# bamler-lab/constriction

Hardware: AMD Instinct MI355X
Metric: Msymbols/s encode+decode, 64k x 4k-symbol streams, bit-exact vs CPU (higher is better)
Workload: dtype u64; 1 GPU; C2: 65536 streams/GPU x 4096 int32 symbols (stream-major), shared 12-bit QuantizedGaussian(-50,50,3.2,9.6), AnsCoder (W,S,P)=(32,64,12), encode into slabs + decode; u64 coder state, u32 words, i32 symbols; streams_per_gpu=65536, parallelism=streams sharded over 1 GPU(s), no data-path collective

## Files before the change

constriction_amd/csrc/cst_family_policy.hpp:

```cpp
#pragma once
#include "cst_math.hpp"
#include "cst_family_math.hpp"

namespace cst {

__device__ __forceinline__ float ndtri_lower_f32(float tail) {
    constexpr float a1 = -3.969683028665376e+01f, a2 = 2.209460984245205e+02f, a3 = -2.759285104469687e+02f, a4 = 1.383577518672690e+02f,
        a5 = -3.066479806614716e+01f, a6 = 2.506628277459239e+00f, b1 = -5.447609879822406e+01f, b2 = 1.615858368580409e+02f,
        b3 = -1.556989798598866e+02f, b4 = 6.680131188771972e+01f, b5 = -1.328068155288572e+01f, c1 = -7.784894002430293e-03f,
        c2 = -3.223964580411365e-01f, c3 = -2.400758277161838e+00f, c4 = -2.549732539343734e+00f, c5 = 4.374664141464968e+00f,
        c6 = 2.938163982698783e+00f, d1 = 7.784695709041462e-03f, d2 = 3.224671290700398e-01f, d3 = 2.445134137142996e+00f,
        d4 = 3.754408661907416e+00f;
    auto f = [](float a, float b, float c) { return __builtin_fmaf(a, b, c); };
    const float q = __builtin_amdgcn_sqrtf(-1.3862943611f * __builtin_amdgcn_logf(tail));
    const float zt = f(f(f(f(f(c1, q, c2), q, c3), q, c4), q, c5), q, c6) * __builtin_amdgcn_rcpf(f(f(f(f(d1, q, d2), q, d3), q, d4), q, 1.0f));
    const float u = tail - 0.5f, r = u * u;
    const float zc = f(f(f(f(f(a1, r, a2), r, a3), r, a4), r, a5), r, a6) * u * __builtin_amdgcn_rcpf(f(f(f(f(f(b1, r, b2), r, b3), r, b4), r, b5), r, 1.0f));
    return tail < 0.02425f ? zt : zc;
}

__device__ __forceinline__ float ndtri_lower_coarse_f32(float tail) {
    const float t = __builtin_amdgcn_sqrtf(-1.3862943611f * __builtin_amdgcn_logf(tail));
    const float num = __builtin_fmaf(__builtin_fmaf(0.010328f, t, 0.802853f), t, 2.515517f);
    const float den = __builtin_fmaf(__builtin_fmaf(__builtin_fmaf(0.001308f, t, 0.189269f), t, 1.432788f), t, 1.0f);
    return __builtin_fmaf(num, __builtin_amdgcn_rcpf(den), -t);
}

__device__ __forceinline__ bool family_params_valid(double a, double b) {
    return b > 0.0 && b <= 1.7976931348623157e308 && fabs(a) <= 1.7976931348623157e308;
}

struct GaussianFamily {
    static constexpr bool kGaussian = true, kErfTab = true;
    __device__ static __forceinline__ bool valid(double mu, double sd) { return family_params_valid(mu, sd); }
    __device__ static __forceinline__ bool lcp(int32_t sym, int32_t lo, int32_t hi, int P, double mu, double sd, uint32_t& left, uint32_t& prob,
                                               const double2* tab) {
        return leaky_gaussian_lcp_quick(sym, lo, hi, P, 32, mu, sd, left, prob, tab);
    }
    template <bool INNER = false>
    __device__ static __forceinline__ uint32_t left(int32_t i, int32_t lo, int32_t n, int P, double mu, double sd, const double2* tab) {
        return leaky_gaussian_left_quick<INNER>(i, lo, n, P, 32, mu, sd, tab);
    }
    __device__ static __forceinline__ void left3(uint32_t g, int32_t lo, uint32_t n, int P, double mu, double sd, const double2* tab, uint32_t (&v)[3]) {
        leaky_gaussian_left3_quick(g, lo, n, P, mu, sd, tab, v);
    }
    __device__ static __forceinline__ float guess_z(float tail) { return ndtri_lower_f32(tail); }
    __device__ static __forceinline__ float guess_z_coarse(float tail) { return ndtri_lower_coarse_f32(tail); }
};

static __device__ __attribute__((noinline)) double laplace_left_f64(double x, double mu, double b, double free_weight) {
    return free_weight * laplace_cdf_exact(x, mu, b);
}
static __device__ __attribute__((noinline)) double cauchy_left_f64(double x, double x0, double gamma, double free_weight) {
    return free_weight * cauchy_cdf_exact(x, x0, gamma);
}

template <class CDF>
struct ExactFamily {
    static constexpr bool kGaussian = false, kErfTab = false;
    __device__ static __forceinline__ bool valid(double a, double b) { return family_params_valid(a, b); }
    __device__ static __forceinline__ uint32_t total(int P) { return P >= 32 ? 0u : (1u << P); }
    __device__ static __forceinline__ uint32_t value(uint32_t i, int32_t lo, uint32_t n, int P, double a, double b) {
        const double free_weight = (double)((total(P) - 1u) - (n - 1u));
        const double x = (double)(int32_t)((uint32_t)lo + i) - 0.5;
        return f64_as_u32_hw(CDF::left_f64(x, a, b, free_weight));
    }
    template <bool INNER = false>
    __device__ static __forceinline__ uint32_t left(int32_t i, int32_t lo, int32_t n, int P, double a, double b, const double2*) {
        if constexpr (!INNER) {
            if (i <= 0) return 0u;
            if (i >= n) return total(P);
        }
        return value((uint32_t)i, lo, (uint32_t)n, P, a, b) + (uint32_t)i;
    }
    __device__ static __forceinline__ void left3(uint32_t g, int32_t lo, uint32_t n, int P, double a, double b, const double2*, uint32_t (&v)[3]) {
#pragma unroll 1
        for (uint32_t k = 0; k < 3; ++k) {
            const uint32_t i = g - 1u + k;
            const uint32_t ic = min(max(i, 1u), n - 1u);
            const uint32_t val = value(ic, lo, n, P, a, b) + ic;
            const uint32_t r = i == 0u ? 0u : i >= n ? total(P) : val;
            if (k == 0) v[0] = r; else if (k == 1) v[1] = r; else v[2] = r;
        }
    }
    __device__ static __forceinline__ bool lcp(int32_t sym, int32_t lo, int32_t hi, int P, double a, double b, uint32_t& left_out, uint32_t& prob,
                                               const double2*) {
        const bool inside = sym >= lo && sym <= hi;
        const uint32_t n = (uint32_t)hi - (uint32_t)lo + 1u;
        const uint32_t i = inside ? (uint32_t)sym - (uint32_t)lo : 0u;
        uint32_t e[2];
#pragma unroll 1
        for (uint32_t k = 0; k < 2; ++k) {
            const uint32_t j = i + k;
            const uint32_t jc = min(max(j, 1u), n - 1u);
            const uint32_t val = value(jc, lo, n, P, a, b) + jc;
            const uint32_t r = j == 0u ? 0u : j >= n ? total(P) : val;
            if (k == 0) e[0] = r; else e[1] = r;
        }
        left_out = e[0];
        prob = e[1] - e[0];
        return inside;
    }
    __device__ static __forceinline__ float guess_z(float tail) { return CDF::z(tail); }
    __device__ static __forceinline__ float guess_z_coarse(float tail) { return CDF::z(tail); }
};

struct LaplaceCdf {
    __device__ static __forceinline__ double left_f64(double x, double mu, double b, double fw) { return laplace_left_f64(x, mu, b, fw); }
    __device__ static __forceinline__ float z(float tail) { return 0.69314718f * __builtin_amdgcn_logf(2.0f * tail); }
};
struct CauchyCdf {
    __device__ static __forceinline__ double left_f64(double x, double x0, double g, double fw) { return cauchy_left_f64(x, x0, g, fw); }
    __device__ static __forceinline__ float z(float tail) {
        const float pt = 3.14159265f * tail;
        const float far = __builtin_fmaf(pt, -0.33333333f, __builtin_amdgcn_rcpf(pt));
        const float near = __builtin_amdgcn_cosf(0.5f * tail) * __builtin_amdgcn_rcpf(__builtin_amdgcn_sinf(0.5f * tail));
        return -(tail < 0.03125f ? far : near);
    }
};
using LaplaceFamily = ExactFamily<LaplaceCdf>;
using CauchyFamily = ExactFamily<CauchyCdf>;

}
```

constriction_amd/csrc/cst_math.hpp:

```cpp
#pragma once
#include <hip/hip_runtime.h>
#include <stdint.h>

namespace cst {

__device__ __forceinline__ uint32_t f64_hi(double x) { return (uint32_t)__double2hiint(x); }
__device__ __forceinline__ uint32_t f64_lo(double x) { return (uint32_t)__double2loint(x); }
__device__ __forceinline__ double f64_from(uint32_t lo, uint32_t hi) { return __hiloint2double((int)hi, (int)lo); }
__device__ __forceinline__ double f64_clear_lo(double x) { return __hiloint2double(__double2hiint(x), 0); }
__device__ __forceinline__ double f64_pow2(int n) { return __hiloint2double((0x3ff + n) << 20, 0); }

__device__ inline double scalbn_exact(double x, int n) {
    double y = x;
    if (n > 1023) {
        y *= 0x1p1023; n -= 1023;
        if (n > 1023) { y *= 0x1p1023; n -= 1023; if (n > 1023) n = 1023; }
    } else if (n < -1022) {
        y *= 0x1p-1022 * 0x1p53; n += 1022 - 53;
        if (n < -1022) { y *= 0x1p-1022 * 0x1p53; n += 1022 - 53; if (n < -1022) n = -1022; }
    }
    return y * f64_pow2(n);
}

__device__ inline double exp_exact(double x) {
// ... 247 lines not shown
}

template <bool TAB = false>
__device__ __forceinline__ uint32_t leaky_gaussian_left(int32_t i, int32_t lo, int32_t n, int P, int prob_bits, double mu,
                                                        double sigma, const double2* tab = nullptr) {
    const uint32_t pmask = prob_bits >= 32 ? 0xffffffffu : ((1u << prob_bits) - 1u);
    if (i <= 0) return 0u;
    if (i >= n) return (P >= 32 ? 0u : (1u << P)) & pmask;
    const uint32_t max_prob = pmask >> (prob_bits - P);
    const double free_weight = (double)(max_prob - (uint32_t)(n - 1));
    const double x = (double)(int32_t)((uint32_t)lo + (uint32_t)i) - 0.5;
    return (f64_as_u32_sat(free_weight * gaussian_cdf_exact<TAB>(x, mu, sigma, tab)) + (uint32_t)i) & pmask;
}

static __device__ __attribute__((noinline)) double leaky_left_f64_exact(double x, double mu, double sigma, double free_weight, const double2* tab) {
    constexpr double sqrt2 = 1.41421356237309504880168872420969808;
    return free_weight * ((1.0 + erf_exact_tab((x - mu) / (sigma * sqrt2), tab)) / 2.0);
}

__device__ __forceinline__ uint32_t leaky_left_value_quick(double x, double mu, double sigma, double inv_d, double free_weight,
                                                           const double2* tab, uint32_t* n_exact) {
    constexpr double sqrt2 = 1.41421356237309504880168872420969808;
    const double arg = (x - mu) * inv_d;
    const double half = 0.5 * free_weight;
    double y = __builtin_fma(erf_fast_poly(arg, tab), half, half);
    const double fr = __builtin_amdgcn_fract(y);
    const bool same = __builtin_fabs(arg) >= 6.0;
    const bool sure = __builtin_fabs(fr - 0.5) < 0.5 - kLeftGuard;
    const bool unsure = !(same || sure);
    if (__builtin_amdgcn_ballot_w64(unsure) != 0ull) {
        if (unsure) {
            y = leaky_left_f64_exact(x, mu, sigma, free_weight, tab);
            if (n_exact) ++*n_exact;
        }
    }
    return f64_as_u32_hw(y);
}

template <bool INNER = false>
__device__ __forceinline__ uint32_t leaky_gaussian_left_quick(int32_t i, int32_t lo, int32_t n, int P, int prob_bits, double mu,
                                                              double sigma, const double2* tab, uint32_t* n_exact = nullptr) {
    constexpr double sqrt2 = 1.41421356237309504880168872420969808;
    const uint32_t pmask = prob_bits >= 32 ? 0xffffffffu : ((1u << prob_bits) - 1u);
    if constexpr (!INNER) {
        if (i <= 0) return 0u;
        if (i >= n) return (P >= 32 ? 0u : (1u << P)) & pmask;
    }
    const uint32_t max_prob = pmask >> (prob_bits - P);
    const double free_weight = (double)(max_prob - (uint32_t)(n - 1));
    const double x = (double)(int32_t)((uint32_t)lo + (uint32_t)i) - 0.5;
    return (leaky_left_value_quick(x, mu, sigma, fast_rcp1(sigma * sqrt2), free_weight, tab, n_exact) + (uint32_t)i) & pmask;
}

__device__ __forceinline__ void leaky_gaussian_left3_quick(uint32_t g, int32_t lo, uint32_t n, int P, double mu, double sigma,
                                                           const double2* tab, uint32_t (&v)[3]) {
    constexpr double sqrt2 = 1.41421356237309504880168872420969808;
    const uint32_t total = P >= 32 ? 0u : (1u << P);
    const double free_weight = (double)((total - 1u) - (n - 1u));
    const double half = 0.5 * free_weight;
    const double inv_d = fast_rcp1(sigma * sqrt2);
    const double x1 = (double)(int32_t)((uint32_t)lo + g) - 0.5;
    const double x[3] = {x1 - 1.0, x1, x1 + 1.0};
    double y[3], arg[3];
    bool unsure[3];
    ErfPoly e[3];
#pragma unroll
    for (int k = 0; k < 3; ++k) {
        arg[k] = (x[k] - mu) * inv_d;
        e[k] = erf_poly_fetch(arg[k], tab);
    }
    __builtin_amdgcn_sched_barrier(0);
#pragma unroll
    for (int k = 0; k < 3; ++k) {
        y[k] = __builtin_fma(erf_poly_eval(e[k], arg[k]), half, half);
        unsure[k] = !(__builtin_fabs(arg[k]) >= 6.0 || __builtin_fabs(__builtin_amdgcn_fract(y[k]) - 0.5) < 0.5 - kLeftGuard);
    }
    unsure[0] = unsure[0] && g > 1u;
    unsure[2] = unsure[2] && g + 1u < n;
    if (__builtin_amdgcn_ballot_w64(unsure[0] || unsure[1] || unsure[2]) != 0ull) {
#pragma unroll
        for (int k = 0; k < 3; ++k)
            if (unsure[k]) y[k] = leaky_left_f64_exact(x[k], mu, sigma, free_weight, tab);
    }
    v[0] = g > 1u ? f64_as_u32_hw(y[0]) + (g - 1u) : 0u;
    v[1] = f64_as_u32_hw(y[1]) + g;
    v[2] = g + 1u < n ? f64_as_u32_hw(y[2]) + (g + 1u) : total;
}

__device__ __forceinline__ bool leaky_gaussian_lcp_quick(int32_t sym, int32_t lo, int32_t hi, int P, int prob_bits, double mu, double sigma,
                                                         uint32_t& left, uint32_t& prob, const double2* tab) {
    constexpr double sqrt2 = 1.41421356237309504880168872420969808;
    const bool inside = sym >= lo && sym <= hi;
    const int32_t sc = inside ? sym : lo;
    const uint32_t pmask = prob_bits >= 32 ? 0xffffffffu : ((1u << prob_bits) - 1u);
    const uint32_t max_prob = pmask >> (prob_bits - P);
    const double free_weight = (double)(max_prob - ((uint32_t)hi - (uint32_t)lo));
    const double half = 0.5 * free_weight;
    const uint32_t slack = ((uint32_t)sc - (uint32_t)lo) & pmask;
    const double inv_d = fast_rcp1(sigma * sqrt2);
    const double xl = (double)sc - 0.5, xr = (double)sc + 0.5;
    const double al = (xl - mu) * inv_d, ar = (xr - mu) * inv_d;
    const ErfPoly el = erf_poly_fetch(al, tab), er = erf_poly_fetch(ar, tab);
    __builtin_amdgcn_sched_barrier(0);
    double yl = __builtin_fma(erf_poly_eval(el, al), half, half), yr = __builtin_fma(erf_poly_eval(er, ar), half, half);
    const bool unsure_l = !(__builtin_fabs(al) >= 6.0 || __builtin_fabs(__builtin_amdgcn_fract(yl) - 0.5) < 0.5 - kLeftGuard) && sc != lo;
    const bool unsure_r = !(__builtin_fabs(ar) >= 6.0 || __builtin_fabs(__builtin_amdgcn_fract(yr) - 0.5) < 0.5 - kLeftGuard) && sc != hi;
    if (__builtin_amdgcn_ballot_w64(unsure_l || unsure_r) != 0ull) {
#pragma unroll 1
        for (int side = 0; side < 2; ++side) {
            const bool u = side ? unsure_r : unsure_l;
            if (__builtin_amdgcn_ballot_w64(u) == 0ull) continue;
            if (u) {
                const double y = leaky_left_f64_exact(side ? xr : xl, mu, sigma, free_weight, tab);
                if (side) yr = y; else yl = y;
            }
        }
    }
    const uint32_t l = sc == lo ? 0u : (f64_as_u32_hw(yl) + slack) & pmask;
    const uint32_t r = sc == hi ? ((P >= 32 ? 0u : (1u << P)) & pmask) : (f64_as_u32_hw(yr) + slack + 1u) & pmask;
    left = l;
    prob = (r - l) & pmask;
    return inside;
}

}
```

constriction_amd/csrc/cst_persymbol.hip:

```cpp
#include <cstdlib>
#include <mutex>

#include "cst_persymbol.hpp"

namespace cst {

__global__ void cp_entries_kernel(const uint32_t* __restrict__ left, const uint32_t* __restrict__ prob, size_t n, int P,
                                  EncEntry* __restrict__ out) {
    const size_t i = (size_t)blockIdx.x * blockDim.x + threadIdx.x;
    if (i >= n) return;
    uint32_t c = left[i], p = prob[i];
    if ((uint64_t)c + p > ((uint64_t)1 << P)) p = 0;
    out[i] = make_entry(c, p);
}

template <int W, int S, int KIND>
__global__ __launch_bounds__(kBlock) void encode_entries_kernel(const EntriesEncodeArgs a) {
    extern __shared__ __attribute__((aligned(16))) unsigned char smem[];
    const int lane = threadIdx.x & (kWave - 1);
    uint32_t* ring = reinterpret_cast<uint32_t*>(smem) + (threadIdx.x >> 6) * kRingWords;
    const size_t s = (size_t)blockIdx.x * blockDim.x + threadIdx.x;
    const bool active = s < a.n_streams;
    const size_t N = a.n_per_stream;
    const int P = a.precision;
// ... 264 lines not shown
}

__device__ __noinline__ void store_symbol_tile16(int32_t* sym, size_t n_streams, size_t N, size_t s0, size_t t0, int lane, const int32_t* tile, bool vec) {
#pragma unroll
    for (int k = 0; k < 4; ++k) {
        const size_t r = (size_t)(lane >> 2) + 16 * k;
        if (s0 + r >= n_streams) continue;
        const int32_t* src = tile + r * 20 + 4 * (lane & 3);
        int32_t* dst = sym + (s0 + r) * N + t0 + 4 * (lane & 3);
        if (vec) {
            const int4 v = *reinterpret_cast<const int4*>(src);
            v4i t; t.x = v.x; t.y = v.y; t.z = v.z; t.w = v.w;
            __builtin_nontemporal_store(t, reinterpret_cast<v4i*>(dst));
        } else {
            dst[0] = src[0]; dst[1] = src[1]; dst[2] = src[2]; dst[3] = src[3];
        }
    }
}

template <class PT> __device__ __forceinline__ size_t edge_row_length(size_t n) {
    if constexpr (kParamF32<PT>) asm volatile("" : "+s"(n));
    return n;
}

template <int W, int S, int KIND, bool SMALL = false, class FAM = GaussianFamily, class PT = double>
__global__ __launch_bounds__(LaneGeo<SMALL>::kThreads) void decode_gaussian_lane_kernel(const PerSymbolDecodeArgs a) {
    using G = LaneGeo<SMALL>;
    constexpr int kParTile = G::kParTile, kWordWindow = G::kWordWindow, kOutSyms = G::kOutSyms, kOutStride = G::kOutStride;
    constexpr size_t kLaneDecWaveBytes = G::kWaveBytes;
    extern __shared__ __attribute__((aligned(16))) unsigned char smem[];
    double2* erf_tab = reinterpret_cast<double2*>(smem);
    if constexpr (FAM::kErfTab) {
        erf_tab_fill(erf_tab, threadIdx.x, blockDim.x);
        __syncthreads();
    }
    const int lane = threadIdx.x & (kWave - 1);
    unsigned char* mine = smem + (FAM::kErfTab ? kErfTabBytes : 0) + (size_t)(threadIdx.x >> 6) * kLaneDecWaveBytes;
    int32_t* tile = reinterpret_cast<int32_t*>(mine);
    double* par_mu = reinterpret_cast<double*>(mine + (size_t)kWave * kOutStride * 4);
    double* par_sd = par_mu + kParTile * kParStride;
    uint32_t* win = reinterpret_cast<uint32_t*>(par_sd + kParTile * kParStride);
    const size_t s = (size_t)blockIdx.x * blockDim.x + threadIdx.x;
    const size_t s0 = s - lane;
    if (s0 >= a.n_streams) return;
    const bool active = s < a.n_streams;
    const size_t se = active ? s : a.n_streams - 1;
    const size_t N = a.n_per_stream;
    const int P = a.precision;
    const bool raw = (a.flags & CST_FLAG_RAW_STATE) != 0;
    const uint32_t n = (uint32_t)a.n_symbols;
    const bool symbol_major = a.layout == CST_LAYOUT_SYMBOL_MAJOR;
    const size_t stride_t = symbol_major ? a.n_streams : 1;
    const size_t e0 = symbol_major ? se : se * N;
    const double free_weight = (double)((P >= 32 ? 0xffffffffu : ((1u << P) - 1u)) - (n - 1u));
    const float total_f = (float)(1ull << P), free_f = (float)free_weight, inv_total_f = 1.0f / total_f, inv_free_f = 1.0f / free_f;
    const double guess_shift = 0.5 - (double)a.min_symbol;
    const bool vec = !symbol_major && (N % 4 == 0) && (reinterpret_cast<uintptr_t>(a.symbols) & 15) == 0;
    const bool two_step_guess = (double)n * 64.0 > free_weight;

    DirectDecoder<W, S, KIND> D;
    D.init(a, se, raw);
    int32_t status = D.status;
    int32_t* sym_p = a.symbols + e0;

    constexpr int kVec = !kParamF32<PT> ? 1 : SMALL ? 2 : KIND != kRange ? 4 : 1;
    constexpr int kReqTile = kParamsPerLine<PT>;
    constexpr int kReqParts = kReqTile / kParTile;
    constexpr bool kMulti = kReqParts > 1;
    PT mu_r[kReqTile], sd_r[kReqTile];
    const PT* const means = params_as<PT>(a.means);
    const PT* const stds = params_as<PT>(a.stds);
    int mode = 0;
    const size_t base_e = symbol_major ? s0 + (size_t)lane : (s0 + (size_t)(lane / kParTile)) * N + (size_t)(lane % kParTile);
    const size_t t_stride = symbol_major ? a.n_streams : 1, item_stride = symbol_major ? a.n_streams : (size_t)(kWave / kParTile) * N;
    const int base_l = symbol_major ? lane : (lane % kParTile) * kParStride + lane / kParTile;
    const int l_stride = symbol_major ? kParStride : kWave / kParTile;
    const bool vec_ok = kVec == 1 || (N % kVec == 0 && ((reinterpret_cast<uintptr_t>(means) | reinterpret_cast<uintptr_t>(stds)) & (4 * kVec - 1)) == 0);
    const bool pairs = kMulti && !symbol_major && s0 + kWave <= a.n_streams && vec_ok;
    constexpr int kLanesPerRow = kReqTile / kVec;
    typedef float vec_t __attribute__((ext_vector_type(kVec > 1 ? kVec : 2)));
    auto par_request = [&](size_t t0) {
        if (kMulti && pairs && t0 % kReqTile == 0 && t0 + kReqTile <= N) {
            if constexpr (kVec > 1) {
                const size_t ev = (s0 + (size_t)(lane / kLanesPerRow)) * N + (size_t)(kVec * (lane % kLanesPerRow)) + t0;
#pragma unroll
                for (int it = 0; it < kLanesPerRow; ++it) {
                    const vec_t mv = __builtin_nontemporal_load(reinterpret_cast<const vec_t*>(means + ev + (size_t)it * (kWave / kLanesPerRow) * N));
                    const vec_t sv = __builtin_nontemporal_load(reinterpret_cast<const vec_t*>(stds + ev + (size_t)it * (kWave / kLanesPerRow) * N));
#pragma unroll
                    for (int c = 0; c < kVec; ++c) { mu_r[kVec * it + c] = mv[c]; sd_r[kVec * it + c] = sv[c]; }
                }
                mode = 1;
                return;
            }
            const size_t e = (s0 + (size_t)(lane / kReqTile)) * N + (size_t)(lane % kReqTile) + t0;
            const PT* pm = means + e;
            const PT* ps = stds + e;
#pragma unroll
            for (int it = 0; it < kReqTile; ++it) {
                mu_r[it] = __builtin_nontemporal_load(pm + (size_t)it * (size_t)(kWave / kReqTile) * N);
                sd_r[it] = __builtin_nontemporal_load(ps + (size_t)it * (size_t)(kWave / kReqTile) * N);
            }
            mode = 1;
            return;
        }
        mode = 0;
        if (s0 + kWave <= a.n_streams && t0 + kParTile <= N) {
            const PT* pm = means + base_e + t0 * t_stride;
            const PT* ps = stds + base_e + t0 * t_stride;
#pragma unroll
            for (int it = 0; it < kParTile; ++it) {
// ... 45 lines not shown
            par_mu[base_l + it * l_stride] = (double)mu_r[it];
            par_sd[base_l + it * l_stride] = (double)sd_r[it];
        }
    };
    uint32_t w_r[kParTile];
    int64_t w_first = 0;
    auto win_request = [&](int64_t first) {
        w_first = first;
        const int64_t len = (int64_t)D.length();
        if (!__any(first < 0 || first + kParTile > len)) {
            const uint32_t* pw = D.in + first;
#pragma unroll
            for (int i = 0; i < kParTile; ++i) w_r[i] = pw[i];
            return;
        }
#pragma unroll
        for (int i = 0; i < kParTile; ++i) {
            const int64_t p = first + i;
            w_r[i] = *(p >= 0 && p < len ? D.in + p : D.idle);
        }
    };
    auto win_land = [&]() {
#pragma unroll
        for (int i = 0; i < kParTile; ++i) win[(((uint32_t)(w_first + i)) & (kWordWindow - 1)) * kWave + lane] = w_r[i];
    };
    const auto window_of = [&](int ahead_tiles) -> int64_t {
        return D.kDownward ? (int64_t)D.position() - (int64_t)kParTile * (ahead_tiles + 1) : (int64_t)D.position() + (int64_t)kParTile * ahead_tiles;
    };

    if (N > 0) {
        par_request(0);
        win_request(window_of(0));
    }
    for (size_t t0 = 0; t0 < N; t0 += kParTile) {
        wave_lds_fence();
        par_land();
        win_land();
        if (t0 + kParTile < N && mode == 0) par_request(t0 + kParTile);
        win_request(window_of(1));
        wave_lds_fence();
        const int n_here = (int)(N - t0 < (size_t)kParTile ? N - t0 : (size_t)kParTile);
#pragma unroll 1
        for (int tl = 0; tl < n_here; ++tl) {
            const size_t t = t0 + (size_t)tl;
            int32_t sym = 0;
            const double mu = par_mu[tl * kParStride + lane], sd = par_sd[tl * kParStride + lane];
            D.ahead = win[(((uint32_t)D.next_index()) & (kWordWindow - 1)) * kWave + lane];
            if (status == CST_STREAM_OK) {
                const bool model_ok = FAM::valid(mu, sd);
                const uint32_t q = model_ok ? D.quantile(P) : 0u;
                if (!model_ok) status = CST_STREAM_IMPOSSIBLE_SYMBOL;
                else if (D.status != CST_STREAM_OK) status = D.status;
                else {
                    const float below = (float)q + 0.5f, above = total_f - below;
                    const bool coarse = FAM::kGaussian && !__any(sd >= 200.0);
                    float z = coarse ? FAM::guess_z_coarse(fminf(below, above) * inv_total_f) : FAM::guess_z(fminf(below, above) * inv_total_f);
                    double x = mu + sd * (double)(below < above ? z : -z) + guess_shift;
                    if (two_step_guess) {
                        const float b1 = below - (float)fmin(fmax(x, 0.0), (double)(n - 1u)), a1 = free_f - b1;
                        z = FAM::guess_z(fmaxf(fminf(b1, a1), 0.25f) * inv_free_f);
                        x = mu + sd * (double)(b1 < a1 ? z : -z) + guess_shift;
                    }
                    const uint32_t g = (uint32_t)fmin(fmax(x + 0.5, 1.0), (double)(n - 1u));
                    uint32_t lo_i = 0, hi_i = n, lo_v = 0, hi_v = P >= 32 ? 0u : (1u << P);
                    uint32_t probe = g, step = 1;
                    bool up = false, down = false;
                    {
                        uint32_t v3[3];
                        FAM::left3(g, a.min_symbol, n, P, mu, sd, erf_tab, v3);
                        if (v3[1] <= q) {
                            up = true;
                            if (q < v3[2]) { lo_i = g; lo_v = v3[1]; hi_i = g + 1u; hi_v = v3[2]; }
                            else { lo_i = g + 1u; lo_v = v3[2]; probe = min(g + 2u, n - 1u); step = 2; }
                        } else {
                            down = true;
                            if (v3[0] <= q) { lo_i = g - 1u; lo_v = v3[0]; hi_i = g; hi_v = v3[1]; }
                            else { hi_i = g - 1u; hi_v = v3[0]; probe = max(g - 1u, 2u) - 1u; step = 2; }
                        }
                    }
                    while (hi_i - lo_i > 1) {
                        const uint32_t v = FAM::template left<true>((int32_t)probe, a.min_symbol, (int32_t)n, P, mu, sd, erf_tab);
                        if (v <= q) { lo_i = probe; lo_v = v; up = true; } else { hi_i = probe; hi_v = v; down = true; }
                        if (up && down) probe = lo_i + (hi_i - lo_i) / 2;
                        else if (up) probe = min(lo_i + step, hi_i - 1u);
                        else probe = max(hi_i - min(step, hi_i - 1u), lo_i + 1u);
                        step *= 2;
                    }
                    const uint32_t c = lo_v, p = hi_v - lo_v;
                    if (p == 0 || c > q || (uint64_t)c + p > ((uint64_t)1 << P)) status = CST_STREAM_IMPOSSIBLE_SYMBOL;
                    else {
                        sym = a.min_symbol + (int32_t)lo_i;
                        D.advance(q, c, p, P);
                    }
                }
            }
            if (symbol_major) {
                if (active) *sym_p = sym;
                sym_p += stride_t;
            } else {
                tile[lane * kOutStride + (t % kOutSyms)] = sym;
                if (t % kOutSyms == kOutSyms - 1) {
                    wave_lds_fence();
                    if constexpr (SMALL) store_symbol_tile16(a.symbols, a.n_streams, N, s0, t - (kOutSyms - 1), lane, tile, vec);
                    else store_symbol_tile(a.symbols, a.n_streams, N, s0, t - (kOutSyms - 1), lane, tile, vec);
                    wave_lds_fence();
                }
            }
        }
    }
    if (!symbol_major) {
        const size_t done = N - N % kOutSyms;
        if (active) for (size_t t = done; t < N; ++t) a.symbols[se * N + t] = tile[lane * kOutStride + (t % kOutSyms)];
    }
    if (!active) return;
    a.status[s] = status;
    D.finish(a, s, raw);
}

constexpr int kRowsAhead = 16;

template <class FAM = GaussianFamily, class PT = double>
__global__ __launch_bounds__(kRowEntries) void gaussian_rows_kernel(int P, int32_t lo, int32_t n, const PT* __restrict__ means,
                                                                   const PT* __restrict__ stds, int32_t layout, size_t n_streams,
                                                                   size_t N, size_t t0, size_t count, uint32_t* __restrict__ rows) {
    const double2* erf_tab = nullptr;
    if constexpr (FAM::kErfTab) {
        __shared__ double2 erf_lds[kErfTabEntries];
        erf_tab_fill(erf_lds, threadIdx.x, blockDim.x);
        __syncthreads();
        erf_tab = erf_lds;
    }
    const size_t row = blockIdx.x;
    const size_t s = row / count, t = t0 + row % count;
    const size_t e = layout == CST_LAYOUT_SYMBOL_MAJOR ? t * n_streams + s : s * N + t;
    const double mu = load_param(means + e), sd = load_param(stds + e);
    const int32_t i = (int32_t)threadIdx.x;
    const uint32_t total = 1u << P;
    uint32_t v;
    if (FAM::valid(mu, sd))
        v = i <= n ? FAM::template left<false>(i, lo, n, P, mu, sd, erf_tab) : total;
    else v = i == 0 ? 0xffffffffu : total;
    rows[row * kRowEntries + i] = v;
}

// ... 891 lines not shown
```

constriction_amd/csrc/cst_persymbol.hpp:

```cpp
#pragma once
#include <type_traits>

#include "cst_range_kernels.hpp"
#include "cst_math.hpp"
#include "cst_family_policy.hpp"

namespace cst {

enum CoderKind : int { kAns = 0, kRange = 1, kChain = 2 };

template <class PT> __device__ __forceinline__ const PT* params_as(const void* p) { return static_cast<const PT*>(p); }
template <class PT> __device__ __forceinline__ double load_param(const PT* p) { return (double)*p; }
template <class PT> inline constexpr bool kParamF32 = std::is_same_v<PT, float>;
template <class PT> inline constexpr int kParamsPerLine = 128 / (int)sizeof(PT);

inline const float* f32(const void* p) { return static_cast<const float*>(p); }

__device__ __forceinline__ EncEntry make_entry(uint32_t c, uint32_t p) {
    uint64_t m = 0;
    if (p == 1) m = ~0ull;
    else if (p > 1) {
        const uint64_t q = (~0ull) / p;
        const uint64_t r = (~0ull) - q * p;
        m = q + ((r + 1 == p) ? 1 : 0);
    }
    return EncEntry{c, p, (uint32_t)m, (uint32_t)(m >> 32)};
}

struct EntriesEncodeArgs {
    const EncEntry* entries;
    size_t n_streams, n_per_stream;
    int32_t layout, precision;
    uint32_t* words;
    size_t stride_words;
    uint32_t* n_words;
    uint64_t* state;
    cst_range_state* rstate;
    int32_t* status;
    uint32_t flags;
    const uint32_t* pop_words; const uint64_t* pop_offsets; size_t pop_stride; uint32_t* n_pop;
    cst_chain_heads* heads;
};

constexpr int kEntryGroup = 8;

constexpr int kFuTile = 16;
constexpr int kFuStreams = 32;
constexpr int kFuIters = kFuTile * kFuStreams / kWave;
constexpr int kFuRingSlots = 32;
constexpr int kFuAhead = 4;
constexpr int kFuRowStride = kFuStreams + 1;
constexpr int kFuBlock = 256;
constexpr size_t kFuTabBytes = kErfTabBytes;
constexpr size_t kFuWaveBytes = (size_t)kFuRingSlots * kWave * 4 + (size_t)kFuTile * kFuRowStride * sizeof(EncEntry);

__device__ __forceinline__ EncEntry make_entry_f64(uint32_t c, uint32_t p) {
    const uint32_t pp = p > 1u ? p : 2u;
    const double inv = fast_rcp1((double)pp);
// ... 346 lines not shown
```

constriction_amd/csrc/cst_persymbol_ragged.hpp:

```cpp
#pragma once
#include "cst_persymbol.hpp"

namespace cst {


__device__ __forceinline__ size_t persymbol_ragged_stream(const uint32_t* order, size_t slot, size_t n_streams, bool& active) {
    active = slot < n_streams;
    if (!active || !order) return slot;
    const size_t s = order[slot];
    active = s < n_streams;
    return s;
}

__device__ __forceinline__ uint32_t persymbol_wave_max(uint32_t v) {
#pragma unroll
    for (int d = 32; d >= 1; d >>= 1) v = max(v, (uint32_t)__shfl_xor((int)v, d));
    return (uint32_t)__builtin_amdgcn_readfirstlane((int)v);
}

struct GaussianRaggedEncodeArgs {
    const int32_t* symbols;
    const void* means;
    const void* stds;
    const uint64_t* sym_offsets;
// ... 259 lines not shown
        const uint64_t out = ((uint64_t)(uint32_t)__shfl((int)out_hi, r) << 32) | (uint64_t)(uint32_t)__shfl((int)out_lo, r);
        const uint64_t n = (uint64_t)(uint32_t)__shfl((int)len, r), sk = (uint64_t)(uint32_t)__shfl((int)skip, r);
        const uint64_t tp = t0 + 4u * (uint32_t)(lane & 3);
        if (tp >= n || tp + 4 <= sk) continue;
        const int32_t* src = tile + r * 20 + 4 * (lane & 3);
        if (tp >= sk && tp + 4 <= n) {
            const int4 v = *reinterpret_cast<const int4*>(src);
            v4i t; t.x = v.x; t.y = v.y; t.z = v.z; t.w = v.w;
            reinterpret_cast<v4i_at4*>(sym + out + (tp - sk))->v = t;
        } else {
#pragma unroll
            for (int i = 0; i < 4; ++i)
                if (tp + (uint64_t)i >= sk && tp + (uint64_t)i < n) sym[out + (tp + (uint64_t)i - sk)] = src[i];
        }
    }
}

template <int W, int S, int KIND, class FAM = GaussianFamily, int MODE = kRgPlain, class PT = double>
__global__ __launch_bounds__(kRgDecThreads) void decode_gaussian_ragged_kernel(const GaussianRaggedDecodeArgsOf<MODE> ra) {
    static_assert(KIND == kAns || KIND == kRange, "a stack or a queue");
    using G = LaneGeo<true>;
    constexpr int kParTile = G::kParTile, kWordWindow = G::kWordWindow, kOutSyms = G::kOutSyms, kOutStride = G::kOutStride;
    static_assert(kOutSyms == 16 && kOutStride == 20, "store_symbol_tile_ragged's tile");
    const PerSymbolDecodeArgs& a = ra.p;
    extern __shared__ __attribute__((aligned(16))) unsigned char smem[];
    double2* erf_tab = reinterpret_cast<double2*>(smem);
    if constexpr (FAM::kErfTab) {
        erf_tab_fill(erf_tab, threadIdx.x, blockDim.x);
        __syncthreads();
    }
    const int lane = threadIdx.x & (kWave - 1);
    unsigned char* mine = smem + (FAM::kErfTab ? kErfTabBytes : 0) + (size_t)(threadIdx.x >> 6) * G::kWaveBytes;
    int32_t* tile = reinterpret_cast<int32_t*>(mine);
    double* par_mu = reinterpret_cast<double*>(mine + (size_t)kWave * kOutStride * 4);
    double* par_sd = par_mu + kParTile * kParStride;
    uint32_t* win = reinterpret_cast<uint32_t*>(par_sd + kParTile * kParStride);
    const size_t slot = (size_t)blockIdx.x * blockDim.x + threadIdx.x;
    if (slot - lane >= a.n_streams) return;
    bool active;
    const size_t s = ragged_lane_stream<MODE>(ra, slot, a.n_streams, active);
    const size_t se = active ? s : 0;
    const uint64_t sym_lo = active ? ragged_lane_begin<MODE>(ra, s) : 0, sym_hi = active ? ragged_lane_end<MODE>(ra, s) : 0;
    const bool too_long = sym_hi - sym_lo > 0xffffffffull || sym_hi < sym_lo;
    const uint32_t len = too_long ? 0u : (uint32_t)(sym_hi - sym_lo);
    const uint32_t off_lo = (uint32_t)sym_lo, off_hi = (uint32_t)(sym_lo >> 32);
    uint32_t out_lo = 0, out_hi = 0, skip = 0;
    if constexpr (MODE == kRgSelect) {
        const uint64_t o = active ? ra.out_lo[s] : 0;
        out_lo = (uint32_t)o; out_hi = (uint32_t)(o >> 32); skip = active ? ra.skip[s] : 0u;
    }
    const uint64_t mx = persymbol_wave_max(len);
    const int P = a.precision;
    const uint32_t n = (uint32_t)a.n_symbols;
    const double free_weight = (double)((P >= 32 ? 0xffffffffu : ((1u << P) - 1u)) - (n - 1u));
    const float total_f = (float)(1ull << P), free_f = (float)free_weight, inv_total_f = 1.0f / total_f, inv_free_f = 1.0f / free_f;
    const double guess_shift = 0.5 - (double)a.min_symbol;
    const bool two_step_guess = (double)n * 64.0 > free_weight;

    DirectDecoder<W, S, KIND> D;
    D.init(a, se, ragged_lane_raw<MODE>(ra));
    int32_t status = D.status;

    PT mu_r[kParTile], sd_r[kParTile];
    const PT* const means = params_as<PT>(a.means);
    const PT* const stds = params_as<PT>(a.stds);
    const int item_t = lane & (kParTile - 1), item_j0 = lane / kParTile;
    auto par_request = [&](uint64_t t0) {
#pragma unroll
        for (int it = 0; it < kParTile; ++it) {
            const int j = it * (kWave / kParTile) + item_j0;
            const uint64_t off = ((uint64_t)(uint32_t)__shfl((int)off_hi, j) << 32) | (uint64_t)(uint32_t)__shfl((int)off_lo, j);
            const uint64_t t = t0 + (uint64_t)item_t;
            const uint64_t e = t < (uint64_t)(uint32_t)__shfl((int)len, j) ? off + t : 0;
            mu_r[it] = __builtin_nontemporal_load(means + e);
            sd_r[it] = __builtin_nontemporal_load(stds + e);
        }
    };
    auto par_land = [&]() {
#pragma unroll
        for (int it = 0; it < kParTile; ++it) {
            par_mu[item_t * kParStride + it * (kWave / kParTile) + item_j0] = (double)mu_r[it];
            par_sd[item_t * kParStride + it * (kWave / kParTile) + item_j0] = (double)sd_r[it];
        }
    };
    constexpr bool kDownward = DirectDecoder<W, S, KIND>::kDownward;
    uint32_t w_r[kParTile];
    int64_t w_first = 0;
    auto win_request = [&](int64_t first) {
        w_first = first;
        if constexpr (kDownward) {
            if (!__any(first < 0)) {
                const uint32_t* pw = D.in + first;
#pragma unroll
                for (int i = 0; i < kParTile; ++i) w_r[i] = pw[i];
                return;
            }
#pragma unroll
            for (int i = 0; i < kParTile; ++i) {
                const int64_t p = first + i;
                w_r[i] = *(p >= 0 ? D.in + p : D.idle);
            }
        } else {
            const int64_t len = (int64_t)D.length();
            if (!__any(first < 0 || first + kParTile > len)) {
                const uint32_t* pw = D.in + first;
#pragma unroll
                for (int i = 0; i < kParTile; ++i) w_r[i] = pw[i];
                return;
            }
#pragma unroll
            for (int i = 0; i < kParTile; ++i) {
                const int64_t p = first + i;
                w_r[i] = *(p >= 0 && p < len ? D.in + p : D.idle);
            }
        }
    };
    auto win_land = [&]() {
#pragma unroll
        for (int i = 0; i < kParTile; ++i) win[(((uint32_t)(w_first + i)) & (kWordWindow - 1)) * kWave + lane] = w_r[i];
    };
    const auto window_of = [&](int ahead_tiles) -> int64_t {
        if constexpr (kDownward) return (int64_t)D.position() - (int64_t)kParTile * (ahead_tiles + 1);
        else return (int64_t)D.position() + (int64_t)kParTile * ahead_tiles;
    };

    if (mx > 0) {
        par_request(0);
        win_request(window_of(0));
    }
    for (uint64_t t0 = 0; t0 < mx; t0 += kParTile) {
        wave_lds_fence();
        par_land();
        win_land();
        if (t0 + kParTile < mx) par_request(t0 + kParTile);
        win_request(window_of(1));
        wave_lds_fence();
        const int n_wave = (int)(mx - t0 < (uint64_t)kParTile ? mx - t0 : (uint64_t)kParTile);
#pragma unroll 1
        for (int tl = 0; tl < n_wave; ++tl) {
            const uint64_t t = t0 + (uint64_t)tl;
            int32_t sym = 0;
            const double mu = par_mu[tl * kParStride + lane], sd = par_sd[tl * kParStride + lane];
            D.ahead = win[(((uint32_t)D.next_index()) & (kWordWindow - 1)) * kWave + lane];
            if (t < (uint64_t)len && status == CST_STREAM_OK) {
                const bool model_ok = FAM::valid(mu, sd);
                const uint32_t q = model_ok ? D.quantile(P) : 0u;
                if (!model_ok) status = CST_STREAM_IMPOSSIBLE_SYMBOL;
                else if (D.status != CST_STREAM_OK) status = D.status;
                else {
                    const float below = (float)q + 0.5f, above = total_f - below;
                    const bool coarse = FAM::kGaussian && !__any(sd >= 200.0);
                    float z = coarse ? FAM::guess_z_coarse(fminf(below, above) * inv_total_f) : FAM::guess_z(fminf(below, above) * inv_total_f);
                    double x = mu + sd * (double)(below < above ? z : -z) + guess_shift;
                    if (two_step_guess) {
                        const float b1 = below - (float)fmin(fmax(x, 0.0), (double)(n - 1u)), a1 = free_f - b1;
                        z = FAM::guess_z(fmaxf(fminf(b1, a1), 0.25f) * inv_free_f);
                        x = mu + sd * (double)(b1 < a1 ? z : -z) + guess_shift;
                    }
                    const uint32_t g = (uint32_t)fmin(fmax(x + 0.5, 1.0), (double)(n - 1u));
                    uint32_t lo_i = 0, hi_i = n, lo_v = 0, hi_v = P >= 32 ? 0u : (1u << P);
                    uint32_t probe = g, step = 1;
                    bool up = false, down = false;
                    {
                        uint32_t v3[3];
                        FAM::left3(g, a.min_symbol, n, P, mu, sd, erf_tab, v3);
                        if (v3[1] <= q) {
                            up = true;
                            if (q < v3[2]) { lo_i = g; lo_v = v3[1]; hi_i = g + 1u; hi_v = v3[2]; }
                            else { lo_i = g + 1u; lo_v = v3[2]; probe = min(g + 2u, n - 1u); step = 2; }
                        } else {
                            down = true;
                            if (v3[0] <= q) { lo_i = g - 1u; lo_v = v3[0]; hi_i = g; hi_v = v3[1]; }
                            else { hi_i = g - 1u; hi_v = v3[0]; probe = max(g - 1u, 2u) - 1u; step = 2; }
                        }
                    }
                    while (hi_i - lo_i > 1) {
                        const uint32_t v = FAM::template left<true>((int32_t)probe, a.min_symbol, (int32_t)n, P, mu, sd, erf_tab);
                        if (v <= q) { lo_i = probe; lo_v = v; up = true; } else { hi_i = probe; hi_v = v; down = true; }
                        if (up && down) probe = lo_i + (hi_i - lo_i) / 2;
                        else if (up) probe = min(lo_i + step, hi_i - 1u);
                        else probe = max(hi_i - min(step, hi_i - 1u), lo_i + 1u);
                        step *= 2;
                    }
                    const uint32_t c = lo_v, p = hi_v - lo_v;
                    if (p == 0 || c > q || (uint64_t)c + p > ((uint64_t)1 << P)) status = CST_STREAM_IMPOSSIBLE_SYMBOL;
                    else {
                        sym = a.min_symbol + (int32_t)lo_i;
                        D.advance(q, c, p, P);
                    }
                }
            }
            tile[lane * kOutStride + (int)(t % kOutSyms)] = sym;
            if (t % kOutSyms == kOutSyms - 1) {
                wave_lds_fence();
                if constexpr (MODE == kRgSelect) store_symbol_tile_select(a.symbols, out_lo, out_hi, skip, len, t - (kOutSyms - 1), lane, tile);
                else store_symbol_tile_ragged(a.symbols, off_lo, off_hi, len, t - (kOutSyms - 1), lane, tile);
                wave_lds_fence();
            }
        }
    }
    if (mx % kOutSyms != 0) {
        wave_lds_fence();
        if constexpr (MODE == kRgSelect) store_symbol_tile_select(a.symbols, out_lo, out_hi, skip, len, mx - mx % kOutSyms, lane, tile);
        else store_symbol_tile_ragged(a.symbols, off_lo, off_hi, len, mx - mx % kOutSyms, lane, tile);
    }
    if (!active) return;
    a.status[s] = too_long ? (int32_t)CST_STREAM_CAPACITY : status;
}

inline cst_status check_ragged_gaussian_args(cst_coder_config cfg, int32_t min_symbol, int32_t max_symbol, const void* d_symbols, const void* d_means,
                                             const void* d_stds, const void* d_sym_offsets, const void* d_words, const void* d_word_offsets,
                                             size_t stride_words, const void* d_n_words, const void* d_status, const void* d_order, size_t n_streams) {
    if (!d_symbols || !d_means || !d_stds || !d_sym_offsets || !d_words || !d_n_words || !d_status) return CST_ERR_INVALID_ARGUMENT;
    if (!config_supported(cfg) || max_symbol <= min_symbol) return CST_ERR_INVALID_ARGUMENT;
    if (!d_word_offsets && stride_words == 0) return CST_ERR_INVALID_ARGUMENT;
    if (d_order && n_streams > 0xffffffffull) return CST_ERR_INVALID_ARGUMENT;
    if (support_too_large(cfg, min_symbol, max_symbol)) return CST_ERR_MODEL;
    return CST_OK;
}


struct PerSymbolJumpScratch {
    uint64_t* sym_lo; uint64_t* word_off; uint64_t* state; cst_range_state* rstate;
    uint32_t* len; uint32_t* n_words; uint32_t* owner; int32_t* status;
    PerSymbolJumpScratch(void* d_scratch, size_t n) {
        unsigned char* b = reinterpret_cast<unsigned char*>((reinterpret_cast<uintptr_t>(d_scratch) + 15) & ~(uintptr_t)15);
        rstate = reinterpret_cast<cst_range_state*>(b);
        sym_lo = reinterpret_cast<uint64_t*>(rstate + n); word_off = sym_lo + n; state = word_off + n;
        len = reinterpret_cast<uint32_t*>(state + n); n_words = len + n; owner = n_words + n;
        status = reinterpret_cast<int32_t*>(owner + n);
    }
};
static_assert(sizeof(cst_range_state) == 40, "the scratch layout above");
constexpr uint32_t kPjNoOwner = 0xffffffffu;

template <int W, int S, int KIND>
__global__ void persymbol_jump_chunks_kernel(const uint32_t* __restrict__ words, const uint64_t* __restrict__ sym_offsets,
                                             const uint64_t* __restrict__ word_offsets, size_t stride_words, uint64_t words_capacity,
                                             const uint32_t* __restrict__ n_words, const uint64_t* __restrict__ chunk_offsets, size_t n_streams,
                                             size_t n_chunks_total, uint32_t interval, const uint32_t* __restrict__ jump_pos,
// ... 103 lines not shown
```

Measured before the change: 533,200 Msymbols/s.

## Replace three-point decode bracket with two-point guess and wave-skipped search

Decoder symbol search now evaluates the CDF at two points (the guessed symbol and the one after it) instead of three. It skips the expanding search entirely when no lane in the wave misses the bracket. The coarse inverse-normal guess is dropped in favour of the accurate one, so a better initial guess makes a two-point check sufficient more often. The exact-fallback evaluation is now serialized per side with a per-side ballot. The search logic is moved into a shared SymbolSearch helper used by both the regular and ragged kernels. The trade-off is a costlier guess per symbol and longer searches whenever the guess misses.

```diff
diff --git a/constriction_amd/csrc/cst_family_policy.hpp b/constriction_amd/csrc/cst_family_policy.hpp
--- a/constriction_amd/csrc/cst_family_policy.hpp
+++ b/constriction_amd/csrc/cst_family_policy.hpp
@@ -19,13 +19,6 @@
     return tail < 0.02425f ? zt : zc;
 }
 
-__device__ __forceinline__ float ndtri_lower_coarse_f32(float tail) {
-    const float t = __builtin_amdgcn_sqrtf(-1.3862943611f * __builtin_amdgcn_logf(tail));
-    const float num = __builtin_fmaf(__builtin_fmaf(0.010328f, t, 0.802853f), t, 2.515517f);
-    const float den = __builtin_fmaf(__builtin_fmaf(__builtin_fmaf(0.001308f, t, 0.189269f), t, 1.432788f), t, 1.0f);
-    return __builtin_fmaf(num, __builtin_amdgcn_rcpf(den), -t);
-}
-
 __device__ __forceinline__ bool family_params_valid(double a, double b) {
     return b > 0.0 && b <= 1.7976931348623157e308 && fabs(a) <= 1.7976931348623157e308;
 }
@@ -41,11 +34,10 @@
     __device__ static __forceinline__ uint32_t left(int32_t i, int32_t lo, int32_t n, int P, double mu, double sd, const double2* tab) {
         return leaky_gaussian_left_quick<INNER>(i, lo, n, P, 32, mu, sd, tab);
     }
-    __device__ static __forceinline__ void left3(uint32_t g, int32_t lo, uint32_t n, int P, double mu, double sd, const double2* tab, uint32_t (&v)[3]) {
-        leaky_gaussian_left3_quick(g, lo, n, P, mu, sd, tab, v);
+    __device__ static __forceinline__ void left2(uint32_t j, int32_t lo, uint32_t n, int P, double mu, double sd, const double2* tab, uint32_t (&v)[2]) {
+        leaky_gaussian_left2_quick(j, lo, n, P, mu, sd, tab, v);
     }
     __device__ static __forceinline__ float guess_z(float tail) { return ndtri_lower_f32(tail); }
-    __device__ static __forceinline__ float guess_z_coarse(float tail) { return ndtri_lower_coarse_f32(tail); }
 };
 
 static __device__ __attribute__((noinline)) double laplace_left_f64(double x, double mu, double b, double free_weight) {
@@ -73,36 +65,27 @@
         }
         return value((uint32_t)i, lo, (uint32_t)n, P, a, b) + (uint32_t)i;
     }
-    __device__ static __forceinline__ void left3(uint32_t g, int32_t lo, uint32_t n, int P, double a, double b, const double2*, uint32_t (&v)[3]) {
+    __device__ static __forceinline__ void left2(uint32_t j, int32_t lo, uint32_t n, int P, double a, double b, const double2*, uint32_t (&v)[2]) {
 #pragma unroll 1
-        for (uint32_t k = 0; k < 3; ++k) {
-            const uint32_t i = g - 1u + k;
+        for (uint32_t k = 0; k < 2; ++k) {
+            const uint32_t i = j + k;
             const uint32_t ic = min(max(i, 1u), n - 1u);
             const uint32_t val = value(ic, lo, n, P, a, b) + ic;
             const uint32_t r = i == 0u ? 0u : i >= n ? total(P) : val;
-            if (k == 0) v[0] = r; else if (k == 1) v[1] = r; else v[2] = r;
+            if (k == 0) v[0] = r; else v[1] = r;
         }
     }
     __device__ static __forceinline__ bool lcp(int32_t sym, int32_t lo, int32_t hi, int P, double a, double b, uint32_t& left_out, uint32_t& prob,
                                                const double2*) {
         const bool inside = sym >= lo && sym <= hi;
         const uint32_t n = (uint32_t)hi - (uint32_t)lo + 1u;
-        const uint32_t i = inside ? (uint32_t)sym - (uint32_t)lo : 0u;
         uint32_t e[2];
-#pragma unroll 1
-        for (uint32_t k = 0; k < 2; ++k) {
-            const uint32_t j = i + k;
-            const uint32_t jc = min(max(j, 1u), n - 1u);
-            const uint32_t val = value(jc, lo, n, P, a, b) + jc;
-            const uint32_t r = j == 0u ? 0u : j >= n ? total(P) : val;
-            if (k == 0) e[0] = r; else e[1] = r;
-        }
+        left2(inside ? (uint32_t)sym - (uint32_t)lo : 0u, lo, n, P, a, b, nullptr, e);
         left_out = e[0];
         prob = e[1] - e[0];
         return inside;
     }
     __device__ static __forceinline__ float guess_z(float tail) { return CDF::z(tail); }
-    __device__ static __forceinline__ float guess_z_coarse(float tail) { return CDF::z(tail); }
 };
 
 struct LaplaceCdf {
diff --git a/constriction_amd/csrc/cst_math.hpp b/constriction_amd/csrc/cst_math.hpp
--- a/constriction_amd/csrc/cst_math.hpp
+++ b/constriction_amd/csrc/cst_math.hpp
@@ -323,39 +323,33 @@
     return (leaky_left_value_quick(x, mu, sigma, fast_rcp1(sigma * sqrt2), free_weight, tab, n_exact) + (uint32_t)i) & pmask;
 }
 
-__device__ __forceinline__ void leaky_gaussian_left3_quick(uint32_t g, int32_t lo, uint32_t n, int P, double mu, double sigma,
-                                                           const double2* tab, uint32_t (&v)[3]) {
+__device__ __forceinline__ void leaky_gaussian_left2_quick(uint32_t j, int32_t lo, uint32_t n, int P, double mu, double sigma,
+                                                           const double2* tab, uint32_t (&v)[2]) {
     constexpr double sqrt2 = 1.41421356237309504880168872420969808;
     const uint32_t total = P >= 32 ? 0u : (1u << P);
     const double free_weight = (double)((total - 1u) - (n - 1u));
     const double half = 0.5 * free_weight;
     const double inv_d = fast_rcp1(sigma * sqrt2);
-    const double x1 = (double)(int32_t)((uint32_t)lo + g) - 0.5;
-    const double x[3] = {x1 - 1.0, x1, x1 + 1.0};
-    double y[3], arg[3];
-    bool unsure[3];
-    ErfPoly e[3];
-#pragma unroll
-    for (int k = 0; k < 3; ++k) {
-        arg[k] = (x[k] - mu) * inv_d;
-        e[k] = erf_poly_fetch(arg[k], tab);
-    }
+    const double xl = (double)(int32_t)((uint32_t)lo + j) - 0.5, xr = xl + 1.0;
+    const double al = (xl - mu) * inv_d, ar = (xr - mu) * inv_d;
+    const ErfPoly el = erf_poly_fetch(al, tab), er = erf_poly_fetch(ar, tab);
     __builtin_amdgcn_sched_barrier(0);
-#pragma unroll
-    for (int k = 0; k < 3; ++k) {
-        y[k] = __builtin_fma(erf_poly_eval(e[k], arg[k]), half, half);
-        unsure[k] = !(__builtin_fabs(arg[k]) >= 6.0 || __builtin_fabs(__builtin_amdgcn_fract(y[k]) - 0.5) < 0.5 - kLeftGuard);
-    }
-    unsure[0] = unsure[0] && g > 1u;
-    unsure[2] = unsure[2] && g + 1u < n;
-    if (__builtin_amdgcn_ballot_w64(unsure[0] || unsure[1] || unsure[2]) != 0ull) {
-#pragma unroll
-        for (int k = 0; k < 3; ++k)
-            if (unsure[k]) y[k] = leaky_left_f64_exact(x[k], mu, sigma, free_weight, tab);
-    }
-    v[0] = g > 1u ? f64_as_u32_hw(y[0]) + (g - 1u) : 0u;
-    v[1] = f64_as_u32_hw(y[1]) + g;
-    v[2] = g + 1u < n ? f64_as_u32_hw(y[2]) + (g + 1u) : total;
+    double yl = __builtin_fma(erf_poly_eval(el, al), half, half), yr = __builtin_fma(erf_poly_eval(er, ar), half, half);
+    const bool unsure_l = !(__builtin_fabs(al) >= 6.0 || __builtin_fabs(__builtin_amdgcn_fract(yl) - 0.5) < 0.5 - kLeftGuard) && j > 0u;
+    const bool unsure_r = !(__builtin_fabs(ar) >= 6.0 || __builtin_fabs(__builtin_amdgcn_fract(yr) - 0.5) < 0.5 - kLeftGuard) && j + 1u < n;
+    if (__builtin_amdgcn_ballot_w64(unsure_l || unsure_r) != 0ull) {
+#pragma unroll 1
+        for (int side = 0; side < 2; ++side) {
+            const bool u = side ? unsure_r : unsure_l;
+            if (__builtin_amdgcn_ballot_w64(u) == 0ull) continue;
+            if (u) {
+                const double y = leaky_left_f64_exact(side ? xr : xl, mu, sigma, free_weight, tab);
+                if (side) yr = y; else yl = y;
+            }
+        }
+    }
+    v[0] = j > 0u ? f64_as_u32_hw(yl) + j : 0u;
+    v[1] = j + 1u < n ? f64_as_u32_hw(yr) + (j + 1u) : total;
 }
 
 __device__ __forceinline__ bool leaky_gaussian_lcp_quick(int32_t sym, int32_t lo, int32_t hi, int P, int prob_bits, double mu, double sigma,
diff --git a/constriction_amd/csrc/cst_persymbol.hip b/constriction_amd/csrc/cst_persymbol.hip
--- a/constriction_amd/csrc/cst_persymbol.hip
+++ b/constriction_amd/csrc/cst_persymbol.hip
@@ -340,11 +340,8 @@
     const bool symbol_major = a.layout == CST_LAYOUT_SYMBOL_MAJOR;
     const size_t stride_t = symbol_major ? a.n_streams : 1;
     const size_t e0 = symbol_major ? se : se * N;
-    const double free_weight = (double)((P >= 32 ? 0xffffffffu : ((1u << P) - 1u)) - (n - 1u));
-    const float total_f = (float)(1ull << P), free_f = (float)free_weight, inv_total_f = 1.0f / total_f, inv_free_f = 1.0f / free_f;
-    const double guess_shift = 0.5 - (double)a.min_symbol;
     const bool vec = !symbol_major && (N % 4 == 0) && (reinterpret_cast<uintptr_t>(a.symbols) & 15) == 0;
-    const bool two_step_guess = (double)n * 64.0 > free_weight;
+    const SymbolSearch search(P, a.min_symbol, n);
 
     DirectDecoder<W, S, KIND> D;
     D.init(a, se, raw);
@@ -496,44 +493,11 @@
                 if (!model_ok) status = CST_STREAM_IMPOSSIBLE_SYMBOL;
                 else if (D.status != CST_STREAM_OK) status = D.status;
                 else {
-                    const float below = (float)q + 0.5f, above = total_f - below;
-                    const bool coarse = FAM::kGaussian && !__any(sd >= 200.0);
-                    float z = coarse ? FAM::guess_z_coarse(fminf(below, above) * inv_total_f) : FAM::guess_z(fminf(below, above) * inv_total_f);
-                    double x = mu + sd * (double)(below < above ? z : -z) + guess_shift;
-                    if (two_step_guess) {
-                        const float b1 = below - (float)fmin(fmax(x, 0.0), (double)(n - 1u)), a1 = free_f - b1;
-                        z = FAM::guess_z(fmaxf(fminf(b1, a1), 0.25f) * inv_free_f);
-                        x = mu + sd * (double)(b1 < a1 ? z : -z) + guess_shift;
-                    }
-                    const uint32_t g = (uint32_t)fmin(fmax(x + 0.5, 1.0), (double)(n - 1u));
-                    uint32_t lo_i = 0, hi_i = n, lo_v = 0, hi_v = P >= 32 ? 0u : (1u << P);
-                    uint32_t probe = g, step = 1;
-                    bool up = false, down = false;
-                    {
-                        uint32_t v3[3];
-                        FAM::left3(g, a.min_symbol, n, P, mu, sd, erf_tab, v3);
-                        if (v3[1] <= q) {
-                            up = true;
-                            if (q < v3[2]) { lo_i = g; lo_v = v3[1]; hi_i = g + 1u; hi_v = v3[2]; }
-                            else { lo_i = g + 1u; lo_v = v3[2]; probe = min(g + 2u, n - 1u); step = 2; }
-                        } else {
-                            down = true;
-                            if (v3[0] <= q) { lo_i = g - 1u; lo_v = v3[0]; hi_i = g; hi_v = v3[1]; }
-                            else { hi_i = g - 1u; hi_v = v3[0]; probe = max(g - 1u, 2u) - 1u; step = 2; }
-                        }
-                    }
-                    while (hi_i - lo_i > 1) {
-                        const uint32_t v = FAM::template left<true>((int32_t)probe, a.min_symbol, (int32_t)n, P, mu, sd, erf_tab);
-                        if (v <= q) { lo_i = probe; lo_v = v; up = true; } else { hi_i = probe; hi_v = v; down = true; }
-                        if (up && down) probe = lo_i + (hi_i - lo_i) / 2;
-                        else if (up) probe = min(lo_i + step, hi_i - 1u);
-                        else probe = max(hi_i - min(step, hi_i - 1u), lo_i + 1u);
-                        step *= 2;
-                    }
-                    const uint32_t c = lo_v, p = hi_v - lo_v;
+                    uint32_t idx, c, p;
+                    search.template find<FAM>(q, mu, sd, erf_tab, idx, c, p);
                     if (p == 0 || c > q || (uint64_t)c + p > ((uint64_t)1 << P)) status = CST_STREAM_IMPOSSIBLE_SYMBOL;
                     else {
-                        sym = a.min_symbol + (int32_t)lo_i;
+                        sym = a.min_symbol + (int32_t)idx;
                         D.advance(q, c, p, P);
                     }
                 }
diff --git a/constriction_amd/csrc/cst_persymbol.hpp b/constriction_amd/csrc/cst_persymbol.hpp
--- a/constriction_amd/csrc/cst_persymbol.hpp
+++ b/constriction_amd/csrc/cst_persymbol.hpp
@@ -4,6 +4,7 @@
 #include "cst_range_kernels.hpp"
 #include "cst_math.hpp"
 #include "cst_family_policy.hpp"
+#include "cst_persymbol_search.hpp"
 
 namespace cst {
 
diff --git a/constriction_amd/csrc/cst_persymbol_ragged.hpp b/constriction_amd/csrc/cst_persymbol_ragged.hpp
--- a/constriction_amd/csrc/cst_persymbol_ragged.hpp
+++ b/constriction_amd/csrc/cst_persymbol_ragged.hpp
@@ -335,10 +335,7 @@
     const uint64_t mx = persymbol_wave_max(len);
     const int P = a.precision;
     const uint32_t n = (uint32_t)a.n_symbols;
-    const double free_weight = (double)((P >= 32 ? 0xffffffffu : ((1u << P) - 1u)) - (n - 1u));
-    const float total_f = (float)(1ull << P), free_f = (float)free_weight, inv_total_f = 1.0f / total_f, inv_free_f = 1.0f / free_f;
-    const double guess_shift = 0.5 - (double)a.min_symbol;
-    const bool two_step_guess = (double)n * 64.0 > free_weight;
+    const SymbolSearch search(P, a.min_symbol, n);
 
     DirectDecoder<W, S, KIND> D;
     D.init(a, se, ragged_lane_raw<MODE>(ra));
@@ -431,44 +428,11 @@
                 if (!model_ok) status = CST_STREAM_IMPOSSIBLE_SYMBOL;
                 else if (D.status != CST_STREAM_OK) status = D.status;
                 else {
-                    const float below = (float)q + 0.5f, above = total_f - below;
-                    const bool coarse = FAM::kGaussian && !__any(sd >= 200.0);
-                    float z = coarse ? FAM::guess_z_coarse(fminf(below, above) * inv_total_f) : FAM::guess_z(fminf(below, above) * inv_total_f);
-                    double x = mu + sd * (double)(below < above ? z : -z) + guess_shift;
-                    if (two_step_guess) {
-                        const float b1 = below - (float)fmin(fmax(x, 0.0), (double)(n - 1u)), a1 = free_f - b1;
-                        z = FAM::guess_z(fmaxf(fminf(b1, a1), 0.25f) * inv_free_f);
-                        x = mu + sd * (double)(b1 < a1 ? z : -z) + guess_shift;
-                    }
-                    const uint32_t g = (uint32_t)fmin(fmax(x + 0.5, 1.0), (double)(n - 1u));
-                    uint32_t lo_i = 0, hi_i = n, lo_v = 0, hi_v = P >= 32 ? 0u : (1u << P);
-                    uint32_t probe = g, step = 1;
-                    bool up = false, down = false;
-                    {
-                        uint32_t v3[3];
-                        FAM::left3(g, a.min_symbol, n, P, mu, sd, erf_tab, v3);
-                        if (v3[1] <= q) {
-                            up = true;
-                            if (q < v3[2]) { lo_i = g; lo_v = v3[1]; hi_i = g + 1u; hi_v = v3[2]; }
-                            else { lo_i = g + 1u; lo_v = v3[2]; probe = min(g + 2u, n - 1u); step = 2; }
-                        } else {
-                            down = true;
-                            if (v3[0] <= q) { lo_i = g - 1u; lo_v = v3[0]; hi_i = g; hi_v = v3[1]; }
-                            else { hi_i = g - 1u; hi_v = v3[0]; probe = max(g - 1u, 2u) - 1u; step = 2; }
-                        }
-                    }
-                    while (hi_i - lo_i > 1) {
-                        const uint32_t v = FAM::template left<true>((int32_t)probe, a.min_symbol, (int32_t)n, P, mu, sd, erf_tab);
-                        if (v <= q) { lo_i = probe; lo_v = v; up = true; } else { hi_i = probe; hi_v = v; down = true; }
-                        if (up && down) probe = lo_i + (hi_i - lo_i) / 2;
-                        else if (up) probe = min(lo_i + step, hi_i - 1u);
-                        else probe = max(hi_i - min(step, hi_i - 1u), lo_i + 1u);
-                        step *= 2;
-                    }
-                    const uint32_t c = lo_v, p = hi_v - lo_v;
+                    uint32_t idx, c, p;
+                    search.template find<FAM>(q, mu, sd, erf_tab, idx, c, p);
                     if (p == 0 || c > q || (uint64_t)c + p > ((uint64_t)1 << P)) status = CST_STREAM_IMPOSSIBLE_SYMBOL;
                     else {
-                        sym = a.min_symbol + (int32_t)lo_i;
+                        sym = a.min_symbol + (int32_t)idx;
                         D.advance(q, c, p, P);
                     }
                 }
diff --git a/constriction_amd/csrc/cst_persymbol_search.hpp b/constriction_amd/csrc/cst_persymbol_search.hpp
--- /dev/null
+++ b/constriction_amd/csrc/cst_persymbol_search.hpp
@@ -0,0 +1,58 @@
+#pragma once
+#include "cst_family_policy.hpp"
+
+namespace cst {
+
+struct SymbolSearch {
+    int P;
+    int32_t min_symbol;
+    uint32_t n;
+    float total_f, free_f, inv_total_f, inv_free_f;
+    double guess_shift;
+    bool two_step_guess;
+
+    __device__ __forceinline__ SymbolSearch(int precision, int32_t lo, uint32_t n_symbols) : P(precision), min_symbol(lo), n(n_symbols) {
+        const double free_weight = (double)((P >= 32 ? 0xffffffffu : ((1u << P) - 1u)) - (n - 1u));
+        total_f = (float)(1ull << P);
+        free_f = (float)free_weight;
+        inv_total_f = 1.0f / total_f;
+        inv_free_f = 1.0f / free_f;
+        guess_shift = 0.5 - (double)min_symbol;
+        two_step_guess = (double)n * 64.0 > free_weight;
+    }
+
+    template <class FAM>
+    __device__ __forceinline__ void find(uint32_t q, double mu, double sd, const double2* erf_tab, uint32_t& idx, uint32_t& c, uint32_t& p) const {
+        const float below = (float)q + 0.5f, above = total_f - below;
+        float z = FAM::guess_z(fminf(below, above) * inv_total_f);
+        double x = mu + sd * (double)(below < above ? z : -z) + guess_shift;
+        if (two_step_guess) {
+            const float b1 = below - (float)fmin(fmax(x, 0.0), (double)(n - 1u)), a1 = free_f - b1;
+            z = FAM::guess_z(fmaxf(fminf(b1, a1), 0.25f) * inv_free_f);
+            x = mu + sd * (double)(b1 < a1 ? z : -z) + guess_shift;
+        }
+        const uint32_t j = (uint32_t)fmin(fmax(x, 0.0), (double)(n - 1u));
+        uint32_t v2[2];
+        FAM::left2(j, min_symbol, n, P, mu, sd, erf_tab, v2);
+        idx = j; c = v2[0]; p = v2[1] - v2[0];
+        const bool too_high = q < v2[0], too_low = q >= v2[1] && j + 1u < n;
+        if (__any(too_high || too_low)) {
+            uint32_t lo_i = j, hi_i = j + 1u, lo_v = v2[0], hi_v = v2[1];
+            bool up = false, down = false;
+            if (too_high) { lo_i = 0; lo_v = 0; hi_i = j; hi_v = v2[0]; down = true; }
+            if (too_low) { lo_i = j + 1u; lo_v = v2[1]; hi_i = n; hi_v = P >= 32 ? 0u : (1u << P); up = true; }
+            uint32_t probe = too_low ? min(lo_i + 1u, hi_i - 1u) : max(hi_i, 2u) - 1u, step = 2;
+            while (hi_i - lo_i > 1) {
+                const uint32_t v = FAM::template left<true>((int32_t)probe, min_symbol, (int32_t)n, P, mu, sd, erf_tab);
+                if (v <= q) { lo_i = probe; lo_v = v; up = true; } else { hi_i = probe; hi_v = v; down = true; }
+                if (up && down) probe = lo_i + (hi_i - lo_i) / 2;
+                else if (up) probe = min(lo_i + step, hi_i - 1u);
+                else probe = max(hi_i - min(step, hi_i - 1u), lo_i + 1u);
+                step *= 2;
+            }
+            idx = lo_i; c = lo_v; p = hi_v - lo_v;
+        }
+    }
+};
+
+}
```

After: 531,300 Msymbols/s. No clear change (-0.3%).
